# hmc-lair-shark-tracking/auv-sim

Hardware: AMD Instinct MI355X
Metric: RRT-Dubins node expansions/s (RRT.exploring) (higher is better)
Workload: dtype f64; 1 GPU; RRT.exploring 256 obst 200x200 cells 10000 iters x 12288 episodes/GPU, timebin parent sampling; episodes_per_gpu=12288, iters=10000, obstacles=256, cells=40000, parallelism=episodes sharded x1

## Files before the change

auv_sim_amd/csrc/rrt_explore_kernel.h:

```cpp
#ifndef AUVP_RRT_EXPLORE_KERNEL_H
#define AUVP_RRT_EXPLORE_KERNEL_H
#include "auvp_math.h"
#include "auvp_types.h"
#include "auvp_wave.h"

namespace auvp {

constexpr int RRT_WAVES = 4;
constexpr int RRT_X_WAVES = 8;
constexpr int RRT_MAX_CHUNK = 63;
constexpr int RRT_MAX_HAB = 64;
constexpr int RRT_MAX_POLY = 64;
constexpr int RRT_MAX_BINS = 64;
constexpr int RRT_ELIST = 192;

struct RrtTables {
  WorldDev* world;
  RrtParamsDev* params;
  double (*hab)[4];
  double (*poly)[2];
  double (*bins)[2];
};
constexpr int RRT_WORLD_ONLY_BYTES = (int)((sizeof(WorldDev) + 15) & ~(size_t)15);
constexpr int RRT_WORLD_BYTES = RRT_WORLD_ONLY_BYTES + (int)((sizeof(RrtParamsDev) + 15) & ~(size_t)15);
__host__ __device__ inline int rrt_tables_bytes(int n_habitats, int n_poly, int n_bins) {
  return RRT_WORLD_BYTES + n_habitats * 32 + n_poly * 16 + n_bins * 16;
}
__device__ __forceinline__ RrtTables rrt_tables_view(unsigned char* base, int n_habitats, int n_poly) {
  RrtTables t;
  t.world = reinterpret_cast<WorldDev*>(base);
  t.params = reinterpret_cast<RrtParamsDev*>(base + RRT_WORLD_ONLY_BYTES);
  t.hab = reinterpret_cast<double(*)[4]>(base + RRT_WORLD_BYTES);
  t.poly = reinterpret_cast<double(*)[2]>(base + RRT_WORLD_BYTES + n_habitats * 32);
  t.bins = reinterpret_cast<double(*)[2]>(base + RRT_WORLD_BYTES + n_habitats * 32 + n_poly * 16);
  return t;
}
__device__ __forceinline__ void rrt_tables_stage(const RrtTables& S, const WorldDev& W) {
  for (int i = threadIdx.x; i < W.n_habitats; i += blockDim.x) {
    S.hab[i][0] = W.hab[3 * i]; S.hab[i][1] = W.hab[3 * i + 1]; S.hab[i][2] = W.hab[3 * i + 2];
    S.hab[i][3] = W.hab_t[i];
  }
  if (threadIdx.x == 0) *S.world = W;
  for (int i = threadIdx.x; i < W.n_poly * 2; i += blockDim.x) (&S.poly[0][0])[i] = W.poly[i];
  for (int i = threadIdx.x; i < W.n_bins * 2; i += blockDim.x) (&S.bins[0][0])[i] = W.bins[i];
}

struct RrtLdsPlan {
  int chunk;
  int tables, scratch, mt, pts, bins, per_wave, total;
};

__host__ __device__ inline RrtLdsPlan rrt_lds_plan(int K, int max_pts, int nfreq, int obst_slots, int tables_bytes,
                                                   int waves = RRT_X_WAVES) {
  RrtLdsPlan p;
  p.chunk = nfreq < 1 ? 1 : (nfreq > RRT_MAX_CHUNK ? RRT_MAX_CHUNK : nfreq);
  const int C = p.chunk;
  int steer_u = (64 + 3 * C + 3) * 8;
  int steer_s = (7 * ((C + 2) & ~1) + 4) * 8;
  int s = steer_u > steer_s ? steer_u : steer_s;
  p.scratch = (s + 15) & ~15;
  p.mt = 624 * 4;
  p.pts = ((max_pts * 16) + 15) & ~15;
  p.bins = (((K + 2) * 4) + 15) & ~15;
  p.per_wave = p.scratch + p.mt + p.pts + p.bins;
  p.tables = (tables_bytes + 15) & ~15;
  p.total = p.tables + waves * p.per_wave + obst_slots * (3 * 8 + 4);
  return p;
}

__device__ __forceinline__ bool any_point_outside(const double (*poly)[2], int nv, const double (*pts)[2], int n_pts) {
  const int lane = lane_id();
  if (nv <= 0) return n_pts > 0;
  const int per = 64 / nv;
  const int e = lane % nv, pl = lane / nv;
  const int ej = e == 0 ? nv - 1 : e - 1;
  const double xi = poly[e][0], yi = poly[e][1], xj = poly[ej][0], yj = poly[ej][1];
  bool outside = false;
  for (int p0 = 0; p0 < n_pts; p0 += per) {
    const int p = p0 + pl;
    const bool live = pl < per && p < n_pts;
    bool cross = false;
    if (live) {
      const double x = pts[p][0], y = pts[p][1];
      if ((yi > y) != (yj > y)) cross = x < (xj - xi) * (y - yi) / (yj - yi) + xi;
    }
    const unsigned long long cm = wave_ballot(cross);
    const int q = p0 + lane;
    if (lane < per && q < n_pts) {
      const unsigned long long grp = (cm >> (lane * nv)) & (nv == 64 ? ~0ull : ((1ull << nv) - 1ull));
      outside = outside | ((__popcll(grp) & 1) == 0);
    }
  }
  return wave_any(outside);
}

__device__ __forceinline__ int lower_bound_from(const double* __restrict__ a, int n, double v, int i) {
  i = i < 0 ? 0 : (i > n - 1 ? n - 1 : i);
  while (i > 0 && a[i - 1] >= v) i--;
  while (i < n && a[i] < v) i++;
  return i;
}

__device__ __forceinline__ int cell_lookup(const WorldDev& W, double x, double y, const double* grid_lds = nullptr) {
  if (W.n_cells == 0) return -1;
  if (W.sg_enabled && grid_lds) {
    const double *x1 = grid_lds, *x0 = grid_lds + W.sg_ncol, *y1 = x0 + W.sg_ncol, *y0 = y1 + W.sg_nrow;
    int c = (int)auvp_floor((x - W.sg_x1_0) * W.sg_inv_dx) + 1, r = (int)auvp_floor((x - W.sg_y1_0) * W.sg_inv_dy) + 1;
    c = c < 0 ? 0 : (c > W.sg_ncol - 1 ? W.sg_ncol - 1 : c);
    r = r < 0 ? 0 : (r > W.sg_nrow - 1 ? W.sg_nrow - 1 : r);
    const double xc1 = x1[c], xcm = c > 0 ? x1[c - 1] : -__builtin_inf();
    const double yr1 = y1[r], yrm = r > 0 ? y1[r - 1] : -__builtin_inf();
    if (!(xcm < x && xc1 >= x)) c = lower_bound_from(x1, W.sg_ncol, x, c);
    if (!(yrm < x && yr1 >= x)) r = lower_bound_from(y1, W.sg_nrow, x, r);
    if (c >= W.sg_ncol || r >= W.sg_nrow) return -1;
    return (x0[c] <= x && y0[r] <= y) ? r * W.sg_ncol + c : -1;
  }
  if (W.sg_enabled) {
    int gc = (int)auvp_floor((x - W.sg_x1_0) * W.sg_inv_dx) + 1, gr = (int)auvp_floor((x - W.sg_y1_0) * W.sg_inv_dy) + 1;
    gc = gc < 0 ? 0 : (gc > W.sg_ncol - 1 ? W.sg_ncol - 1 : gc);
    gr = gr < 0 ? 0 : (gr > W.sg_nrow - 1 ? W.sg_nrow - 1 : gr);
    const double4 cc = reinterpret_cast<const double4*>(W.sg_col)[gc];
    const double4 rr = reinterpret_cast<const double4*>(W.sg_row)[gr];
    if (cc.x < x && cc.y >= x && rr.x < x && rr.y >= x) return (cc.z <= x && rr.z <= y) ? gr * W.sg_ncol + gc : -1;
    const int c = lower_bound_from(W.sg_x1, W.sg_ncol, x, gc);
    const int r = lower_bound_from(W.sg_y1, W.sg_nrow, x, gr);
    if (c >= W.sg_ncol || r >= W.sg_nrow) return -1;
    if (!(W.sg_x0[c] <= x) || !(W.sg_y0[r] <= y)) return -1;
    return r * W.sg_ncol + c;
  }
  double fb = auvp_floor((x - W.xb_x0) * W.xb_inv_w);
  int b = fb < 0.0 ? 0 : (fb >= (double)W.n_xbuckets ? W.n_xbuckets - 1 : (int)fb);
  if (W.rg_enabled) {
    int lo = W.rg_first[b], hi = W.rg_first[b + 1];
    while (lo < hi) { const int mid = (lo + hi) >> 1; if (W.rg_bp[mid] < x) lo = mid + 1; else hi = mid; }
    const int r = 2 * lo + ((lo < W.n_rg_bp && W.rg_bp[lo] == x) ? 1 : 0);
    const int s = W.rg_off[r], e = W.rg_off[r + 1];
    if (s == e) return -1;
    if (W.rg_pm[s] <= y) return W.rg_id[s];
    if (!(W.rg_pm[e - 1] <= y)) return -1;
    lo = s; hi = e - 1;
    while (hi - lo > 1) { const int mid = (lo + hi) >> 1; if (W.rg_pm[mid] <= y) hi = mid; else lo = mid; }
    return W.rg_id[hi];
  }
  int e = W.xb_off[b + 1];
  for (int k = W.xb_off[b]; k < e; k++) {
    const double4 d = reinterpret_cast<const double4*>(W.xb_data)[k];
    if (y < d.w) return -1;
    if (x >= d.x && x <= d.y && y >= d.z) return W.xb_items[k];
  }
  return -1;
}

struct BinLists {
  int32_t* direct;
  int32_t* over;
  int32_t* dir;
  int n_over, k1;
};

__device__ __forceinline__ BinLists bin_lists(const RrtBuffers& B, size_t episode, int K) {
  BinLists L;
  L.n_over = B.bin_over; L.k1 = K + 1;
  L.direct = B.bin_items + episode * (size_t)B.bin_stride;
  L.over = L.direct + (size_t)L.k1 * AUVP_BIN_HEAD;
  L.dir = L.over + (size_t)L.n_over * 64;
  return L;
}

__device__ __forceinline__ int bin_member(const BinLists& L, int b, int k) {
  if (k < AUVP_BIN_HEAD) return L.direct[b * AUVP_BIN_HEAD + k];
  const int kk = k - AUVP_BIN_HEAD;
  const int chunk = L.dir[(kk >> 6) * L.k1 + b];
  return L.over[chunk * 64 + (kk & 63)];
}

__device__ __forceinline__ int32_t* bin_slot_for_append(const BinLists& L, int b, int c, int& next_chunk, bool writer) {
  if (c < AUVP_BIN_HEAD) return L.direct + (b * AUVP_BIN_HEAD + c);
  const int kk = c - AUVP_BIN_HEAD;
  int32_t* d = L.dir + ((kk >> 6) * L.k1 + b);
  int chunk;
  if ((kk & 63) == 0) {
    if (next_chunk >= L.n_over) return nullptr;
    chunk = next_chunk++;
    if (writer) *d = chunk;
  } else {
    chunk = *d;
  }
  return L.over + (chunk * 64 + (kk & 63));
}

struct CostAcc {
  double c2;
  unsigned long long visited;
  int hits;
};

template <bool LIM = false>
__device__ __forceinline__ void cost_element(const WorldDev& W, const RrtTables& S, int bin_lo, int bin_hi, double w3,
                                             double x, double y, double t, double& tv, int& hab, bool hab_near = true,
                                             const double* grid_lds = nullptr, unsigned long long keep = ~0ull) {
  int tb = -1;
  if (W.bins_sorted) {
    if (bin_hi > bin_lo) {
      int i = (int)auvp_floor((t - W.bins_t1_0) * W.bins_inv_len) + 1;
      i = i < bin_lo ? bin_lo : (i > bin_hi - 1 ? bin_hi - 1 : i);
      const double2 bi = *reinterpret_cast<const double2*>(&S.bins[i][0]);
      const double pm = i > bin_lo ? S.bins[i - 1][1] : -__builtin_inf();
      if (pm < t && bi.y >= t) {
        if (bi.x <= t) tb = i;
      } else {
        while (i > bin_lo && S.bins[i - 1][1] >= t) i--;
        while (i < bin_hi && S.bins[i][1] < t) i++;
        if (i < bin_hi && S.bins[i][0] <= t) tb = i;
      }
    }
  } else {
    for (int b = bin_hi - 1; b >= bin_lo; b--) {
      const double2 r = *reinterpret_cast<const double2*>(&S.bins[b][0]);
      tb = (t >= r.x && t <= r.y) ? b : tb;
    }
  }
  tv = 0.0;
  hab = -1;
  if (tb >= 0) {
    int c = cell_lookup(W, x, y, grid_lds);
    if (c >= 0) tv = w3 * W.prob[(size_t)tb * W.n_cells + c];
    if (hab_near) {
      if (W.hg_n > 0) {
        const double fx = auvp_floor((x - W.hg_x0) * W.hg_inv_w), fy = auvp_floor((y - W.hg_y0) * W.hg_inv_h);
        unsigned long long m = 0ull;
        if (fx >= 0.0 && fy >= 0.0 && fx < (double)W.hg_n && fy < (double)W.hg_n) m = W.hg_mask[(int)fy * W.hg_n + (int)fx];
        if constexpr (LIM) m &= keep;
        while (m) {
          const int h = __ffsll((long long)m) - 1;
          m &= m - 1ull;
          const double2 hxy = *reinterpret_cast<const double2*>(&S.hab[h][0]);
          const double ddx = hxy.x - x, ddy = hxy.y - y;
          if (ddx * ddx + ddy * ddy <= S.hab[h][3]) { hab = h; break; }
        }
      } else {
        for (int h = W.n_habitats - 1; h >= 0; h--) {
          const double2 hxy = *reinterpret_cast<const double2*>(&S.hab[h][0]);
          const double ddx = hxy.x - x, ddy = hxy.y - y;
          if constexpr (LIM) hab = (ddx * ddx + ddy * ddy <= S.hab[h][3] && ((keep >> h) & 1ull)) ? h : hab;
          else hab = (ddx * ddx + ddy * ddy <= S.hab[h][3]) ? h : hab;
        }
      }
    }
  }
}

__device__ __forceinline__ void cost_accumulate(int n_valid, double tv, int hab, double* term, CostAcc& acc) {
  const int lane = lane_id();
  term[lane] = tv;
  unsigned long long hm = wave_ballot(hab >= 0);
  acc.hits += __popcll(hm);
  unsigned long long vis = acc.visited;
  while (hm) {
    int l = __ffsll((long long)hm) - 1;
    int h = __builtin_amdgcn_readlane(hab, l);
    vis |= (1ull << h);
    hm &= ~wave_ballot(hab == h);
  }
  acc.visited = vis;
  wave_sync();
  double c2 = acc.c2;
  for (int i = 0; i < n_valid; i += 8) {
    double2 v[4];
#pragma unroll
    for (int k = 0; k < 4; k++) v[k] = *reinterpret_cast<const double2*>(term + i + 2 * k);
#pragma unroll
    for (int k = 0; k < 4; k++) { c2 = c2 + v[k].x; c2 = c2 + v[k].y; }
  }
  acc.c2 = c2;
  wave_sync();
}

struct CostPre {
  int tb, c, midx;
};
__device__ __forceinline__ CostPre cost_pre(const WorldDev& W, const RrtTables& S, int bin_lo, int bin_hi, double x, double y, double t,
                                            const double* grid_lds) {
  CostPre q;
  q.tb = -1; q.c = -1; q.midx = -1;
  if (W.bins_sorted) {
    if (bin_hi > bin_lo) {
      int i = (int)auvp_floor((t - W.bins_t1_0) * W.bins_inv_len) + 1;
      i = i < bin_lo ? bin_lo : (i > bin_hi - 1 ? bin_hi - 1 : i);
      const double2 bi = *reinterpret_cast<const double2*>(&S.bins[i][0]);
      const double pm = i > bin_lo ? S.bins[i - 1][1] : -__builtin_inf();
      if (pm < t && bi.y >= t) {
        if (bi.x <= t) q.tb = i;
      } else {
        while (i > bin_lo && S.bins[i - 1][1] >= t) i--;
        while (i < bin_hi && S.bins[i][1] < t) i++;
        if (i < bin_hi && S.bins[i][0] <= t) q.tb = i;
      }
    }
  } else {
    for (int b = bin_hi - 1; b >= bin_lo; b--) {
      const double2 r = *reinterpret_cast<const double2*>(&S.bins[b][0]);
      q.tb = (t >= r.x && t <= r.y) ? b : q.tb;
    }
  }
  if (q.tb >= 0) {
    q.c = cell_lookup(W, x, y, grid_lds);
    if (W.hg_n > 0) {
      const double fx = auvp_floor((x - W.hg_x0) * W.hg_inv_w), fy = auvp_floor((y - W.hg_y0) * W.hg_inv_h);
      if (fx >= 0.0 && fy >= 0.0 && fx < (double)W.hg_n && fy < (double)W.hg_n) q.midx = (int)fy * W.hg_n + (int)fx;
    }
  }
  return q;
}
template <bool LIM = false>
__device__ __forceinline__ void cost_post(const WorldDev& W, const RrtTables& S, double w3, double x, double y, const CostPre& q,
                                          double prob, unsigned long long m, double& tv, int& hab, unsigned long long keep = ~0ull) {
  tv = 0.0;
  hab = -1;
  if (q.tb >= 0) {
    if (q.c >= 0) tv = w3 * prob;
    if (W.hg_n > 0) {
      if constexpr (LIM) m &= keep;
      while (m) {
        const int h = __ffsll((long long)m) - 1;
        m &= m - 1ull;
        const double2 hxy = *reinterpret_cast<const double2*>(&S.hab[h][0]);
        const double ddx = hxy.x - x, ddy = hxy.y - y;
        if (ddx * ddx + ddy * ddy <= S.hab[h][3]) { hab = h; break; }
      }
    } else {
      for (int h = W.n_habitats - 1; h >= 0; h--) {
        const double2 hxy = *reinterpret_cast<const double2*>(&S.hab[h][0]);
        const double ddx = hxy.x - x, ddy = hxy.y - y;
        if constexpr (LIM) hab = (ddx * ddx + ddy * ddy <= S.hab[h][3] && ((keep >> h) & 1ull)) ? h : hab;
        else hab = (ddx * ddx + ddy * ddy <= S.hab[h][3]) ? h : hab;
      }
    }
  }
}

__device__ __forceinline__ void cost_pass(const WorldDev& W, const RrtTables& S, int bin_lo, int bin_hi, double w3,
                                          int n_valid, double x, double y, double t, double* term, CostAcc& acc) {
  double tv = 0.0;
  int hab = -1;
  if (lane_id() < n_valid) cost_element(W, S, bin_lo, bin_hi, w3, x, y, t, tv, hab);
  cost_accumulate(n_valid, tv, hab, term, acc);
}

constexpr int RRT_NN_UNROLL = 8;
constexpr int RRT_NN_BLOCK = 64 * RRT_NN_UNROLL;
__host__ __device__ inline long long rrt_nn_stride(int cap_nodes) {
  return ((long long)cap_nodes + RRT_NN_BLOCK - 1) / RRT_NN_BLOCK * RRT_NN_BLOCK;
}

__device__ __forceinline__ int nn_closest(const double2* __restrict__ xy, int n_nodes, double rx, double ry, bool force_exact = false,
                                          int* slow = nullptr) {
  const int lane = lane_id();
  const double inf = __builtin_inf();
  double bd = inf, sd = inf;
  int bt = 0;
  for (int base = 0; base < n_nodes; base += RRT_NN_BLOCK) {
    double2 q[RRT_NN_UNROLL];
#pragma unroll
    for (int u = 0; u < RRT_NN_UNROLL; u++) q[u] = xy[base + u * 64 + lane];
#pragma unroll
    for (int u = 0; u < RRT_NN_UNROLL; u++) {
      const double ddx = rx - q[u].x, ddy = ry - q[u].y;
      const double d2 = ddx * ddx + ddy * ddy;
      const bool lt = d2 < bd;
      sd = (d2 != bd) ? __builtin_fmin(sd, __builtin_fmax(bd, d2)) : sd;
      bd = lt ? d2 : bd;
      bt = lt ? base + u * 64 : bt;
    }
  }
  const double gmin = wave_min_f64(bd);
  const double band = gmin + gmin * 0x1p-49;
  const bool suspect = (bd > gmin && bd <= band) || (sd > gmin && sd <= band);
  int cand = 0x7fffffff;
  const bool exact = wave_any(suspect) || force_exact;
  if (slow) *slow = exact ? 1 : 0;
  if (!exact) {
    const unsigned long long em = wave_ballot(bd == gmin);
    if (__popcll(em) == 1) return uni(__builtin_amdgcn_readlane(bt, __ffsll((long long)em) - 1) + (__ffsll((long long)em) - 1));
    cand = (bd == gmin) ? bt + lane : 0x7fffffff;
  } else {
    double bs = inf;
    for (int m = lane; m < n_nodes; m += 64) {
      const double2 q = xy[m];
      const double ddx = rx - q.x, ddy = ry - q.y;
      const double d = auvp_sqrt(ddx * ddx + ddy * ddy);
      if (d < bs) { bs = d; cand = m; }
    }
    const double smin = wave_min_f64(bs);
    cand = (bs == smin) ? cand : 0x7fffffff;
  }
#pragma unroll
  for (int o = 32; o >= 1; o >>= 1) {
    const int t = __shfl_xor(cand, o, 64);
    cand = t < cand ? t : cand;
  }
  return uni(cand);
}

template <int J, int MODE, bool DIAG>
__global__ __launch_bounds__(RRT_X_WAVES * 64, (MODE == 2 ? (J <= 4 ? 5 : 2) : (J <= 4 ? 6 : 2))) void rrt_explore_kernel(WorldDev W, RrtParamsDev P, RrtBuffers B,
                                                                     int n_episodes, int max_pts) {
  constexpr bool LIM = false;
  constexpr const RrtEpisodeLimDev* lim = nullptr;
#include "rrt_explore_body.h"
}

template <int J>
__global__ __launch_bounds__(RRT_X_WAVES * 64, (J <= 4 ? 6 : 2)) void rrt_explore_lim_kernel(WorldDev W, RrtParamsDev P, RrtBuffers B,
                                                                                           int n_episodes, int max_pts,
                                                                                           const RrtEpisodeLimDev* __restrict__ lim) {
  constexpr int MODE = 0;
  constexpr bool DIAG = false, LIM = true;
#include "rrt_explore_body.h"
}

constexpr int RRT_LEAF_WAVES = 4;
#ifndef AUVP_LEAF_NPL
#define AUVP_LEAF_NPL 2
#endif
#ifndef AUVP_LEAF_WPE
#define AUVP_LEAF_WPE 4
#endif
__host__ __device__ inline int rrt_leaf_grid_lds_bytes(int sg_enabled, int ncol, int nrow) {
  const long long b = 16LL * ((long long)ncol + nrow);
  return (sg_enabled && b <= 48 * 1024) ? (int)b : 0;
}
__host__ __device__ inline int rrt_leaf_mark_words(int cap_nodes) {
  const int w = (cap_nodes + 31) / 32;
  return w <= 4096 ? w : 0;
}

static __global__ __launch_bounds__(RRT_LEAF_WAVES * 64) __attribute__((amdgpu_waves_per_eu(AUVP_LEAF_WPE, AUVP_LEAF_WPE))) void rrt_leaf_kernel(WorldDev W, RrtParamsDev P, RrtBuffers B, int n_episodes,
                                                                      int mark_words) {
  constexpr bool LIM = false;
  constexpr const RrtEpisodeLimDev* lim = nullptr;
#include "rrt_leaf_body.h"
}

static __global__ __launch_bounds__(RRT_LEAF_WAVES * 64) __attribute__((amdgpu_waves_per_eu(AUVP_LEAF_WPE, AUVP_LEAF_WPE))) void rrt_leaf_lim_kernel(
    WorldDev W, RrtParamsDev P, RrtBuffers B, int n_episodes, int mark_words, const RrtEpisodeLimDev* __restrict__ lim) {
  constexpr bool LIM = true;
#include "rrt_leaf_body.h"
}

static __global__ __launch_bounds__(64) void rrt_final_course_kernel(RrtBuffers B, const int64_t* __restrict__ offsets,
                                                              double* __restrict__ out, int n_episodes) {
  const int ep = blockIdx.x;
  if (ep >= n_episodes) return;
  const int lane = lane_id();
  const RrtSummary s = B.summary[ep];
  if (s.best_leaf < 0) return;
  const int capn = B.cap_nodes;
  const size_t capp = (size_t)B.cap_points;
  const double* nodeF = B.node_f + (size_t)ep * capn * 8;
  const int4* nodeI = reinterpret_cast<const int4*>(B.node_i) + (size_t)ep * capn;
  const double* ptF = B.points + (size_t)ep * capp * 6;
  const double* init = B.init + (size_t)ep * 6;
  double* o = out + 7 * (size_t)offsets[ep];
  int pos = s.best_path_len - 1;
  auto node_elem = [&](int m, int at) {
    double* e = o + 7 * (size_t)at;
    const int4 r = nodeI[m];
    if (r.y < 0) {
      e[0] = init[0]; e[1] = init[1]; e[2] = init[2]; e[3] = 0.0; e[4] = init[3]; e[5] = init[4]; e[6] = init[5];
    } else {
      const double* nf = nodeF + (size_t)m * 8;
      e[0] = nf[0]; e[1] = nf[1]; e[2] = nf[2]; e[3] = 0.0; e[4] = nf[3]; e[5] = (double)r.x; e[6] = nf[4];
    }
  };
  if (lane == 0) node_elem(s.best_leaf, pos);
  pos--;
  for (int m = s.best_leaf;;) {
    const int4 r = nodeI[m];
    if (r.y < 0) break;
    const int cnt = r.w, off = r.z;
    for (int k = lane; k < cnt; k += 64) {
      double* e = o + 7 * (size_t)(pos - cnt + 1 + k);
      size_t gi = (size_t)off + k;
      const double* ra = ptF + gi * 3;
      const double* rb = ptF + capp * 3 + gi * 3;
      e[0] = ra[0]; e[1] = ra[1]; e[2] = rb[0]; e[3] = rb[1];
      e[4] = ra[2]; e[5] = (double)r.x; e[6] = rb[2];
    }
    pos -= cnt;
    if (lane == 0) node_elem(r.y, pos);
    pos--;
    m = r.y;
  }
}

}
#endif
```

auv_sim_amd/csrc/rrt_rows_body.h:

```cpp
  extern __shared__ __align__(16) unsigned char smem[];
  const RrtTables S = rrt_tables_view(smem, W.n_habitats, W.n_poly);
  const int wave = (int)(threadIdx.x >> 6);
  const int lane = lane_id();
  const int row = lane >> 4, rl = lane & 15, rowbase = lane & 48;
  const int K = P.K;
  const int wg_waves = (int)(blockDim.x >> 6);
#if AUVP_ROWS_BODY_STREAM
  const RowsStreamLdsPlan plan = rrt_rows_stream_lds_plan(K, RW_MAX_OBST, rrt_tables_bytes(W.n_habitats, W.n_poly, W.n_bins), wg_waves, MIRROR);
  unsigned char* ebase = smem + plan.tables + (size_t)(wave * RW_ROWS + row) * plan.per_ep;
  double* ring = reinterpret_cast<double*>(ebase);
  double* inc = reinterpret_cast<double*>(ebase + plan.ring);
  uint16_t* bin_count = reinterpret_cast<uint16_t*>(ebase + plan.ring + plan.scratch);
#else
  const RowsLdsPlan plan = rrt_rows_lds_plan(K, RW_MAX_OBST, rrt_tables_bytes(W.n_habitats, W.n_poly, W.n_bins), wg_waves);
  unsigned char* ebase = smem + plan.tables + (size_t)(wave * RW_ROWS + row) * plan.per_ep;
  uint32_t* mt = reinterpret_cast<uint32_t*>(ebase);
  double* win = reinterpret_cast<double*>(ebase + plan.mt);
  double* inc = win;
  uint16_t* bin_count = reinterpret_cast<uint16_t*>(ebase + plan.mt + plan.scratch);
#endif

  rrt_tables_stage(S, W);
  if (threadIdx.x == 0) *S.params = P;
  const RrtParamsDev& Q = *S.params;
  double* olx = reinterpret_cast<double*>(smem + plan.tables + (size_t)wg_waves * RW_ROWS * plan.per_ep);
  double* oly = olx + RW_MAX_OBST;
  float* olr = reinterpret_cast<float*>(oly + RW_MAX_OBST);
  for (int i = threadIdx.x; i < RW_MAX_OBST; i += blockDim.x) { olx[i] = W.os_x[i]; oly[i] = W.os_y[i]; olr[i] = W.os_r[i]; }
  __syncthreads();

  const int ep = ((int)blockIdx.x * wg_waves + wave) * RW_ROWS + row;
  bool live = ep < n_episodes;
  const int eps = live ? ep : 0;
  if (!wave_any(live)) return;

  const int capn = B.cap_nodes, capp = B.cap_points, bcap = B.bin_cap;
  double* nodeF = B.node_f + (size_t)eps * capn * 8;
  int4* nodeI = reinterpret_cast<int4*>(B.node_i) + (size_t)eps * capn;
  uint8_t* nodeQ = B.node_q + (size_t)eps * capn;
  double* ptF = B.points + (size_t)eps * capp * 6;
  const BinLists bins = bin_lists(B, (size_t)eps, K);
  int next_chunk = 0;
  const double* init = B.init + (size_t)eps * 6;

#if AUVP_ROWS_BODY_STREAM
  RowStream rng;
  rng.ring = ring;
  rng.src = B.stream + (size_t)eps * (size_t)B.stream_cap;
  rng.pos = 0u; rng.front = 0u; rng.req = 0u;
  rng.cap = (uint32_t)B.stream_cap;
#pragma unroll
  for (int c = 0; c < RS_PEND; c++) rng.pend[c] = rs_piece(0.0);
#ifdef AUVP_STREAM_COUNT_SLOW
  rng.slow = 0u;
#endif
#define ROWS_CONSUME(on, n) stream_advance(rng, on, (uint32_t)(n))
#else
  RowRng rng;
  rng.s = mt;
  for (int i = rl; i < 624; i += 16) mt[i] = B.mt[(size_t)eps * 624 + i];
  {
    int idx = B.mt_index ? B.mt_index[eps] : 624;
    idx = idx < 0 ? 0 : (idx > 624 ? 624 : idx);
    rng.pslot = idx == 624 ? 0u : (uint32_t)idx;
    rng.avail = (uint32_t)(624 - idx);
    rng.drawn = 0ull;
  }
#define ROWS_CONSUME(on, n) rows_advance(rng, on, (uint32_t)(2 * (n)))
#endif
  for (int i = rl; i < K + 2; i += 16) bin_count[i] = 0;
  wave_sync();
  if (live && rl == 0) {
    nodeF[0] = init[0]; nodeF[1] = init[1]; nodeF[2] = init[2]; nodeF[3] = init[3]; nodeF[4] = init[5];
    nodeI[0] = make_int4(0, -1, 0, 0);
    nodeQ[0] = 0;
    bins.direct[(K >= 1 ? 1 : 0) * AUVP_BIN_HEAD] = 0;
    bin_count[K >= 1 ? 1 : 0] = 1;
  }
  wave_sync();
  int n_nodes = 1, n_points = 0, status = 0, n_cand = 0, iters_run = 0;
  double4 sbox_ld = reinterpret_cast<const double4*>(W.os_box)[rl];
  asm volatile("" : "+v"(sbox_ld.x), "+v"(sbox_ld.y), "+v"(sbox_ld.z), "+v"(sbox_ld.w));
  const double4 sbox = sbox_ld;
  typedef const __attribute__((address_space(4))) double* rows_ost_ptr;
  const rows_ost_ptr ost_s = (rows_ost_ptr)W.os_t;
  const int nv_poly = W.n_poly;

  for (int it = 0; it < P.max_iter; it++) {
    if (!wave_any(live)) break;
    int par = 0, n_total = 0, base = 0;
    {
      bool search = live;
      int fo = 0, rb = 0, cnt = 0;
      double u = 0.0;
#if AUVP_ROWS_BODY_STREAM
      StreamBase<MIRROR> sel;
#endif
      for (;;) {
#if AUVP_ROWS_BODY_STREAM
        if (!stream_ensure<MIRROR>(rng, search, 16u, rl) && search) { status = AUVP_ST_STREAM; live = false; iters_run = it; search = false; }
        sel = stream_base<MIRROR>(rng, 0u, rl);
        if (search) u = stream_read(sel, rl, rl);
#else
        rows_ensure(rng, search, 32u, rl);
        if (search) { u = rows_random_at(rng, (uint32_t)rl); win[rl] = u; }
#endif
        const int rbj = (int)py_uniform(1.0, (double)(K + 1), u);
        const bool cand = search && rl < 14;
        const bool badkey = cand && rbj > K;
        const int cj = (cand && !badkey) ? (int)bin_count[rbj] : 0;
        const uint32_t okm = row_ballot(cj != 0, rowbase), badm = row_ballot(badkey, rowbase);
        const int f_ok = okm ? (__ffs((int)okm) - 1) : 16, f_bad = badm ? (__ffs((int)badm) - 1) : 16;
        if (search) {
          if (f_bad < f_ok) { status = -5; live = false; iters_run = it; search = false; }
          else if (f_ok < 16) { fo = f_ok; search = false; }
        }
        const bool again = search;
        ROWS_CONSUME(again, 14);
        const int src = rowbase + (again ? 0 : fo);
        const int rb_n = row_read(rbj, src), cnt_n = row_read(cj, src);
        if (!again && live && cnt == 0) { rb = rb_n; cnt = cnt_n; }
        if (!wave_any(again)) break;
      }
#if AUVP_ROWS_BODY_STREAM
      const double u1 = stream_read(sel, fo + 1, rl), u2 = stream_read(sel, fo + 2, rl);
#else
      wave_sync();
      const double u1 = win[fo + 1], u2 = win[fo + 2];
#endif
      if (live) {
        const int ri = (int)py_uniform(0.0, (double)cnt, u1);
        par = bin_member(bins, rb, ri);
        n_total = (int)auvp_floor(py_uniform(0.0, Q.freq, u2) / 1);
        base = fo + 3;
      }
    }
    const bool on0 = live && 0 < n_total;
    const int n0_ = on0 ? (n_total < RW_C ? n_total : RW_C) : 0;
#if AUVP_ROWS_BODY_STREAM
    if (!stream_ensure<MIRROR>(rng, on0, (uint32_t)(base + 3 * n0_), rl) && on0) { status = AUVP_ST_STREAM; live = false; iters_run = it; }
#else
    auto make_window = [&](bool on, int nwin, int b0) {
      rows_ensure(rng, on, (uint32_t)(2 * (b0 + nwin)), rl);
#pragma unroll
      for (int t = 0; t < 3; t++) {
        const int j = rl + 16 * t;
        if (on && j < nwin) win[j] = rows_random_at(rng, (uint32_t)(b0 + j));
      }
      wave_sync();
    };
    {
      const int e_end = base + 3 * n0_;
      rows_ensure(rng, on0, (uint32_t)(2 * e_end), rl);
#pragma unroll
      for (int t = 0; t < 3; t++) {
        const int e = 16 + rl + 16 * t;
        if (on0 && e < e_end) win[e] = rows_random_at(rng, (uint32_t)e);
      }
      wave_sync();
    }
#endif
    double cx = 0.0, cy = 0.0, cth = 0.0, ctt = 0.0, clen = 0.0;
    if (live) {
      const double2 a = *reinterpret_cast<const double2*>(nodeF + (size_t)par * 8);
      const double2 b = *reinterpret_cast<const double2*>(nodeF + (size_t)par * 8 + 2);
      cx = a.x; cy = a.y; cth = b.x; ctt = b.y;
      clen = nodeF[(size_t)par * 8 + 4];
    }
#if AUVP_ROWS_BODY_STREAM
    stream_top_up<MIRROR>(rng, live, rl);
#endif
    const double px0 = cx, py0 = cy, clen0 = clen;
    int cnt = 0;
    double ptx[2] = {0.0, 0.0}, pty[2] = {0.0, 0.0};
    bool ptv[2] = {false, false};
    bool first_pass = true;
#pragma unroll
    for (int pass = 0; pass < 2; pass++) {
      const int c0 = pass * RW_C;
      const bool on = live && c0 < n_total;
      if (pass != 0 && !wave_any(on)) break;
      const int n = on ? ((n_total - c0) < RW_C ? (n_total - c0) : RW_C) : 0;
      const int nwin = 3 * n;
#ifdef AUVP_ROWS_PAD
      {
        double pd0 = cth, pd1 = cx, pd2 = cy, pd3 = ctt;
#pragma unroll
        for (int q = 0; q < AUVP_ROWS_PAD / 4; q++)
          asm volatile("v_add_f64 %0, %0, 1.0\n\tv_add_f64 %1, %1, 1.0\n\tv_add_f64 %2, %2, 1.0\n\tv_add_f64 %3, %3, 1.0"
                       : "+v"(pd0), "+v"(pd1), "+v"(pd2), "+v"(pd3));
      }
#endif
      const int b0 = first_pass ? base : 0;
#if AUVP_ROWS_BODY_STREAM
      if (pass != 0 && !stream_ensure<MIRROR>(rng, on, (uint32_t)nwin, rl) && on) { status = AUVP_ST_STREAM; live = false; iters_run = it; }
      const StreamBase<MIRROR> wb = stream_base<MIRROR>(rng, (uint32_t)b0, rl);
#define ROWS_WIN(j) stream_read(wb, (j), rl)
#else
      if (pass != 0) make_window(on, nwin, b0);
      const double* wp = win + (pass == 0 ? base : 0);
#define ROWS_WIN(j) wp[j]
#endif
      unsigned long long tpred = 0ull;
#pragma unroll
      for (int t = 0; t < 3; t++) {
        const int j = rl + 16 * t;
        const double dist = py_uniform(0.0, Q.dist_to_end, ROWS_WIN(j));
        const double diff = py_uniform(-Q.diff_max, Q.diff_max, ROWS_WIN(j + 1));
        const unsigned long long fb = __builtin_amdgcn_fcmp(auvp_fabs(dist), auvp_fabs(diff), 2 ) &
                                      __builtin_amdgcn_uicmp((unsigned)(j + 1), (unsigned)nwin, 36 );
        tpred |= ((fb >> rowbase) & 0xffffull) << (16 * t);
      }
      const bool active = rl < n;
      const uint32_t mywin = active ? (uint32_t)(tpred >> (2 * rl)) : 0u;
      const uint32_t below_me = active ? ((1u << rl) - 1u) : 0u;
      int cbelow = active ? rl : 0;
      uint32_t tmask;
      for (;;) {
        const unsigned long long tb = __builtin_amdgcn_uicmp((mywin >> cbelow) & 1u, 0u, 33 );
        tmask = (uint32_t)((tb >> rowbase) & 0xffffull);
        const int cnew = __popc(tmask & below_me);
        const unsigned long long chg = __builtin_amdgcn_uicmp((unsigned)cnew, (unsigned)cbelow, 33 );
        cbelow = cnew;
        if (chg == 0ull) break;
      }
      const int mypos = 2 * rl + cbelow;
      const int used = 2 * n + __popc(tmask);
      const bool taken = (tmask >> rl) & 1u;
      double radius = 0.0, phi = 0.0, vt = 1.0;
      if (taken) {
        const double dist = py_uniform(0.0, Q.dist_to_end, ROWS_WIN(mypos));
        const double diff = py_uniform(-Q.diff_max, Q.diff_max, ROWS_WIN(mypos + 1));
        const double s1 = dist + diff, s2 = dist - diff;
        radius = auvp_div_plain(s1 + s2, -s1 + s2);
        phi = auvp_div_plain(s1 + s2, 2 * radius);
        vt = py_uniform(0.0, 2 * Q.v, ROWS_WIN(mypos + 2));
      }
#undef ROWS_WIN
#if !AUVP_ROWS_BODY_STREAM
      wave_sync();
#endif
      inc[rl] = phi;
      wave_sync();
      const double th = rows_theta_chain(cth, inc);
      const double myth = (rl == 15) ? cth : th;
      double sn, cs;
      auvp_sincos_sk(myth, &sn, &cs);
      double dx = 0.0, dy = 0.0, mv = 0.0, dt = 0.0;
      {
        const uint32_t below = tmask & ((1u << rl) - 1u);
        const int prev = below ? (31 - __clz((int)below)) : 15;
        const double so = row_read_f64(sn, rowbase + prev), co = row_read_f64(cs, rowbase + prev);
        if (taken) {
          dx = radius * (sn - so);
          dy = radius * (-cs + co);
          mv = auvp_sqrt_plain(dx * dx + dy * dy);
          dt = auvp_div_plain(mv, vt);
        }
      }
      if (rl < 15) { inc[rl] = dx; inc[18 + rl] = dy; inc[36 + rl] = dt; inc[54 + rl] = mv; }
      else { inc[15] = 0.0; inc[33] = 0.0; inc[51] = 0.0; inc[69] = 0.0; }
      wave_sync();
      if (rl < 4 && on) {
        double acc = rl == 0 ? cx : (rl == 1 ? cy : (rl == 2 ? ctt : clen));
        double2* rowp = reinterpret_cast<double2*>(inc + rl * 18);
        double2 v[8];
#pragma unroll
        for (int s2 = 0; s2 < 8; s2++) v[s2] = rowp[s2];
#pragma unroll
        for (int s2 = 0; s2 < 8; s2++) { acc = acc + v[s2].x; v[s2].x = acc; acc = acc + v[s2].y; v[s2].y = acc; }
#pragma unroll
        for (int s2 = 0; s2 < 8; s2++) rowp[s2] = v[s2];
      }
      wave_sync();
      double mx = 0.0, my = 0.0, mt_ = 0.0, ml = 0.0;
      if (active) { mx = inc[rl]; my = inc[18 + rl]; mt_ = inc[36 + rl]; ml = inc[54 + rl]; }
      const bool app = taken && (mv >= Q.min_dist);
      const uint32_t amask = row_ballot(app, rowbase);
      const int napp = __popc(amask);
      if (on && (n_points + cnt + napp > capp)) { status = -2; live = false; iters_run = it; }
      const bool wr = app && live;
      if (wr) {
        const int rank = __popc(amask & ((1u << rl) - 1u));
        const size_t gi = (size_t)(n_points + cnt + rank);
        double* ra = ptF + gi * 3;
        double* rb = ptF + (size_t)capp * 3 + gi * 3;
        typedef double nt_f64x2 __attribute__((ext_vector_type(2)));
        nt_f64x2 va, vb; va.x = mx; va.y = my; vb.x = myth; vb.y = vt;
        __builtin_nontemporal_store(va, reinterpret_cast<nt_f64x2*>(ra)); __builtin_nontemporal_store(mt_, ra + 2);
        __builtin_nontemporal_store(vb, reinterpret_cast<nt_f64x2*>(rb)); __builtin_nontemporal_store(ml, rb + 2);
      }
      ptx[pass] = mx; pty[pass] = my; ptv[pass] = wr;
      {
        const int last = n > 0 ? n - 1 : 0;
        const double th_last = row_read_f64(myth, rowbase + last);
        if (on) {
          cnt += napp;
          cx = inc[last]; cy = inc[18 + last]; ctt = inc[36 + last]; clen = inc[54 + last];
          cth = th_last;
        }
      }
      ROWS_CONSUME(on && live, b0 + used);
      first_pass = false;
      wave_sync();
    }
    ROWS_CONSUME(live && n_total == 0, base);

    const double reach = clen - clen0;
    const double bx0 = px0 - reach, by0 = py0 - reach, bx1 = px0 + reach, by1 = py0 + reach;
    const double slack = 0x1p-30 * (auvp_fabs(bx0) + auvp_fabs(bx1) + auvp_fabs(by0) + auvp_fabs(by1) + 1.0);
    const double hx = reach + slack;
    bool hit = false;
    double ex0 = bx0, ey0 = by0, ex1 = bx1, ey1 = by1;
    auto cull_and_test = [&](auto tight_tag) {
      constexpr bool TIGHT = decltype(tight_tag)::value;
      const double hs = hx + slack;
      const bool slot_hit = live && !(sbox.z < px0 - hs || sbox.x > px0 + hs || sbox.w < py0 - hs || sbox.y > py0 + hs);
      uint32_t sm = row_ballot(slot_hit, rowbase);
      double tcx = px0, tcy = py0, thx = hx, thy = hx;
      if (TIGHT) {
        double mnx = px0, mxx = px0, mny = py0, mxy = py0;
#pragma unroll
        for (int q = 0; q < 2; q++) {
          if (ptv[q]) {
            mnx = __builtin_fmin(mnx, ptx[q]); mxx = __builtin_fmax(mxx, ptx[q]);
            mny = __builtin_fmin(mny, pty[q]); mxy = __builtin_fmax(mxy, pty[q]);
          }
        }
        mnx = row_min_f64(mnx); mxx = row_max_f64(mxx); mny = row_min_f64(mny); mxy = row_max_f64(mxy);
        const double ts = 0x1p-30 * (auvp_fabs(mnx) + auvp_fabs(mxx) + auvp_fabs(mny) + auvp_fabs(mxy) + 1.0);
        tcx = (mnx + mxx) * 0.5; tcy = (mny + mxy) * 0.5;
        thx = (mxx - mnx) * 0.5 + ts; thy = (mxy - mny) * 0.5 + ts;
        const bool tight = slot_hit && !(sbox.z < mnx - ts || sbox.x > mxx + ts || sbox.w < mny - ts || sbox.y > mxy + ts);
        sm = row_ballot(tight, rowbase);
        ex0 = mnx; ey0 = mny; ex1 = mxx; ey1 = mxy;
      }
      while (wave_any(sm != 0u)) {
        const bool hs_ = sm != 0u;
        const int j0 = hs_ ? 16 * (__ffs((int)sm) - 1) : 0;
        sm &= sm - 1u;
        const int oi = j0 + rl;
        const double oxj = olx[oi], oyj = oly[oi], orj = (double)olr[oi];
#ifdef AUVP_ROWS_OST_LDS
        const double otj = orj * orj;
#endif
        const bool cand = hs_ && (TIGHT ? !(auvp_fabs(oxj - tcx) > thx + orj || auvp_fabs(oyj - tcy) > thy + orj)
                                        : !(auvp_fabs(oxj - px0) > hx + orj || auvp_fabs(oyj - py0) > hx + orj));
        uint32_t cm = row_ballot(cand, rowbase);
        n_cand += __popc(cm);
        while (wave_any(cm != 0u)) {
          const bool has = cm != 0u;
          const int cl = has ? (__ffs((int)cm) - 1) : 0;
          cm &= cm - 1u;
          const double ox = row_read_f64(oxj, rowbase + cl), oy = row_read_f64(oyj, rowbase + cl);
#ifdef AUVP_ROWS_OST_LDS
          const double ot = row_read_f64(otj, rowbase + cl);
#else
          const int oc = j0 + cl;
          const unsigned long long hasm = __builtin_amdgcn_uicmp((unsigned)has, 0u, 33 );
          double ot = 0.0;
          int rowv = row;
          asm volatile("" : "+v"(rowv));
#pragma unroll
          for (int r = 0; r < RW_ROWS; r++)
            if (hasm & (1ull << (16 * r))) {
              const double t = ost_s[__builtin_amdgcn_readlane(oc, 16 * r)];
              ot = rowv == r ? t : ot;
            }
#endif
#pragma unroll
          for (int q = 0; q < 2; q++) {
            const double ddx = ptx[q] - ox, ddy = pty[q] - oy;
            hit |= has && ptv[q] && (ddx * ddx + ddy * ddy <= ot);
          }
          if (rl == 15) { const double ddx = px0 - ox, ddy = py0 - oy; hit |= has && (ddx * ddx + ddy * ddy <= ot); }
          if (row_ballot(hit, rowbase) != 0u) cm = 0u;
        }
      }
    };
    if (P.flags & AUVP_KFLAG_TIGHT_CULL) cull_and_test(std::true_type{});
    else cull_and_test(std::false_type{});
    const double* sb = S.world->safe_box;
    const bool box_inside = W.has_safe_box && ex0 > sb[0] && ey0 > sb[1] && ex1 < sb[2] && ey1 < sb[3];
    bool outside = false;
    if (wave_any(live && !box_inside)) {
      auto crossing_outside = [&](double x, double y) {
        if (nv_poly <= 0) return true;
        int par_ = 0;
        for (int e = 0; e < nv_poly; e++) {
          const int ej = e == 0 ? nv_poly - 1 : e - 1;
          const double xi = S.poly[e][0], yi = S.poly[e][1], xj = S.poly[ej][0], yj = S.poly[ej][1];
          if ((yi > y) != (yj > y)) par_ ^= (x < (xj - xi) * (y - yi) / (yj - yi) + xi) ? 1 : 0;
        }
        return (par_ & 1) == 0;
      };
      const bool need = live && !box_inside;
#pragma unroll
      for (int q = 0; q < 2; q++)
        if (need && ptv[q]) outside |= crossing_outside(ptx[q], pty[q]);
      if (need && rl == 15) outside |= crossing_outside(px0, py0);
    }
    const bool bad = row_ballot(hit || outside, rowbase) != 0u;
    const bool ok = live && !bad;
    if (ok && n_nodes >= capn) { status = -2; live = false; iters_run = it; }
    const bool acc_ = ok && live;
    const int me = n_nodes;
    if (acc_) {
      double q = auvp_floor(ctt * Q.inv_bin_interval);
      const double r = auvp_fma(-q, Q.bin_interval, ctt);
      if (r < 0.0) q -= 1.0;
      else if (r >= Q.bin_interval) q += 1.0;
      const double fi = q + 1.0;
      const double curr_bin = fi * Q.bin_interval;
      const bool over = curr_bin > Q.max_traj_time;
      bool stored = true;
      if (!over || fi <= (double)K) {
        const int bi = (int)fi;
        const int c = over ? 0 : (int)bin_count[bi];
        int32_t* slot = (c >= bcap || c >= 65535) ? nullptr : bin_slot_for_append(bins, bi, c, next_chunk, rl == 0);
        if (!slot) { status = -2; live = false; iters_run = it; stored = false; }
        else if (rl == 0) { *slot = me; bin_count[bi] = (uint16_t)(c + 1); }
      }
      if (stored) {
        if (rl == 0) {
          double* nf = nodeF + (size_t)me * 8;
          *reinterpret_cast<double2*>(nf) = make_double2(cx, cy);
          *reinterpret_cast<double2*>(nf + 2) = make_double2(cth, ctt);
          nf[4] = clen;
          nodeI[me] = make_int4(it, par, n_points, cnt);
          nodeQ[me] = ctt >= Q.max_traj_time - 30 ? 1 : 0;
        }
        n_nodes++;
        n_points += cnt;
      }
    }
    wave_sync();
  }

  const bool valid = ep < n_episodes;
  if (live) iters_run = P.max_iter;
#if AUVP_ROWS_BODY_STREAM
  const unsigned long long drawn = 2ull * rng.pos;
  if (!stream_ensure<MIRROR>(rng, valid && status == 0, 1u, rl) && valid && status == 0) status = AUVP_ST_STREAM;
  const double after = status == AUVP_ST_STREAM ? 0.0 : stream_read(stream_base<MIRROR>(rng, 0u, rl), rl, rl);
#else
  const unsigned long long drawn = rng.drawn;
  rows_ensure(rng, valid, 2u, rl);
  const double after = rows_random_at(rng, 0u);
#endif
  if (valid) {
    for (int i = rl; i < K + 1; i += 16) B.bin_count[(size_t)ep * (K + 1) + i] = (int32_t)bin_count[i];
    if (rl == 0) {
      RrtSummary& s = B.summary[ep];
#if AUVP_ROWS_BODY_STREAM
      pipe_report(B.pipe_fail, status == AUVP_ST_STREAM ? AUVP_ST_PIPELINE : 0);
#endif
      s.status = status; s.n_nodes = n_nodes; s.n_points = n_points; s.n_leaves = 0;
      s.best_leaf = -1; s.best_path_len = 0; s.iters_run = iters_run; s.n_candidates = n_cand;
      s.best_cost[0] = __builtin_inf(); s.best_cost[1] = 0.0; s.best_cost[2] = 0.0; s.best_cost[3] = 0.0;
      s.best_length = 0.0;
      s.rng_after = after; s.leaf_elems = 0; s.n_draw32 = drawn; s.nn_scanned = 0ull;
#if AUVP_ROWS_BODY_STREAM && defined(AUVP_STREAM_COUNT_SLOW)
      s.nn_scanned = rng.slow;
#endif
    }
  }
#undef ROWS_CONSUME
```

auv_sim_amd/csrc/rrt_rows_stream_kernel.h:

```cpp
#ifndef AUVP_RRT_ROWS_STREAM_KERNEL_H
#define AUVP_RRT_ROWS_STREAM_KERNEL_H
#include "rrt_rows_kernel.h"

namespace auvp {

constexpr int RS_RING = 256;
constexpr int RS_MIRROR = 48;
constexpr int RS_WAVES = 16;
#ifndef AUVP_RS_PIECE
#define AUVP_RS_PIECE 2
#endif
constexpr int RS_PIECE = AUVP_RS_PIECE;
constexpr int RS_CHUNK = 16 * RS_PIECE;
constexpr int RS_PEND = 64 / RS_CHUNK;
typedef double rs_f64x2 __attribute__((ext_vector_type(2)));
template <int N> struct RsPiece { typedef double type; };
template <> struct RsPiece<2> { typedef rs_f64x2 type; };
typedef RsPiece<RS_PIECE>::type rs_piece;
constexpr int RS_LDS_LIMIT = 160 * 1024;

struct RowsStreamLdsPlan {
  int tables, ring, scratch, bins, per_ep, obst, total;
};
__host__ __device__ inline RowsStreamLdsPlan rrt_rows_stream_lds_plan(int K, int n_obst_slots, int tables_bytes, int waves = RW_WAVES, bool mirror = false) {
  RowsStreamLdsPlan p;
  p.tables = (tables_bytes + 15) & ~15;
  p.ring = (RS_RING + (mirror ? RS_MIRROR : 0)) * 8;
  p.scratch = (4 * 18 * 8 + 15) & ~15;
  p.bins = (((K + 2) * 2) + 15) & ~15;
  p.per_ep = p.ring + p.scratch + p.bins;
  p.obst = n_obst_slots * (8 + 8 + 4);
  p.total = p.tables + waves * RW_ROWS * p.per_ep + p.obst;
  return p;
}

struct RowsStreamShape {
  int waves;
  bool mirror;
  RowsStreamLdsPlan plan;
};
__host__ inline RowsStreamShape rrt_rows_stream_shape(int K, int n_obst_slots, int tables_bytes, int waves_wanted, int force = -1) {
  int sw = waves_wanted < 1 ? 1 : (waves_wanted > RW_WAVES ? RW_WAVES : waves_wanted);
  while (sw > 1 && rrt_rows_stream_lds_plan(K, n_obst_slots, tables_bytes, sw, false).total > RS_LDS_LIMIT) sw--;
  bool mirror = force < 0 ? rrt_rows_stream_lds_plan(K, n_obst_slots, tables_bytes, sw, true).total <= RS_LDS_LIMIT : force != 0;
  while (mirror && sw > 1 && rrt_rows_stream_lds_plan(K, n_obst_slots, tables_bytes, sw, true).total > RS_LDS_LIMIT) sw--;
  RowsStreamShape s;
  s.waves = sw; s.mirror = mirror;
  s.plan = rrt_rows_stream_lds_plan(K, n_obst_slots, tables_bytes, sw, mirror);
  return s;
}

struct RowStream {
  double* ring;
  const double* src;
  uint32_t pos, front, req, cap;
  rs_piece pend[RS_PEND];
#ifdef AUVP_STREAM_COUNT_SLOW
  uint32_t slow;
#endif
};

template <bool MIRROR>
__device__ __forceinline__ void stream_commit(RowStream& r, int rl) {
#pragma unroll
  for (int c = 0; c < RS_PEND; c++)
    if (r.front + (uint32_t)(RS_CHUNK * c) < r.req) {
      const uint32_t s = (r.front + (uint32_t)(RS_CHUNK * c) + (uint32_t)(RS_PIECE * rl)) & (uint32_t)(RS_RING - 1);
      *reinterpret_cast<rs_piece*>(r.ring + s) = r.pend[c];
      if (MIRROR && s < (uint32_t)RS_MIRROR) *reinterpret_cast<rs_piece*>(r.ring + s + (uint32_t)RS_RING) = r.pend[c];
    }
  r.front = r.req;
}
__device__ __forceinline__ void stream_request(RowStream& r, bool on, int rl) {
  const uint32_t room = (uint32_t)RS_RING - (r.front - r.pos), left = r.cap - r.req;
  uint32_t n = (room < left ? room : left) / (uint32_t)RS_CHUNK;
  n = n > (uint32_t)RS_PEND ? (uint32_t)RS_PEND : n;
  n = on ? n : 0u;
#pragma unroll
  for (int c = 0; c < RS_PEND; c++)
    if ((uint32_t)c < n)
      r.pend[c] = __builtin_nontemporal_load(reinterpret_cast<const rs_piece*>(r.src + r.req + (uint32_t)(RS_CHUNK * c) + (uint32_t)(RS_PIECE * rl)));
  r.req += (uint32_t)RS_CHUNK * n;
}
__device__ __forceinline__ void stream_settle(RowStream& r) {
#pragma unroll
  for (int c = 0; c < RS_PEND; c++) asm volatile("" : "+v"(r.pend[c]));
}
template <bool MIRROR>
__device__ __forceinline__ void stream_top_up(RowStream& r, bool on, int rl) {
  stream_commit<MIRROR>(r, rl);
  stream_request(r, on, rl);
}
template <bool MIRROR>
__device__ __forceinline__ bool stream_ensure(RowStream& r, bool want, uint32_t need, int rl) {
  const uint32_t need_w = want ? need : 0u;
  const bool ok = r.pos + need_w <= r.cap;
  for (;;) {
    if (__builtin_amdgcn_uicmp(r.front - r.pos, ok ? need_w : 0u, 36 ) == 0ull) break;
    const bool go = ok && r.front - r.pos < need_w;
#ifdef AUVP_STREAM_COUNT_SLOW
    if (go) r.slow++;
#endif
    stream_commit<MIRROR>(r, rl);
    stream_request(r, go && ok, rl);
    stream_commit<MIRROR>(r, rl);
    stream_settle(r);
    wave_sync();
    if (!wave_any(go && ok && r.front - r.pos < need_w)) break;
  }
  wave_sync();
  return ok;
}
template <bool MIRROR> struct StreamBase;
template <> struct StreamBase<true> { const double* p; };
template <> struct StreamBase<false> { const double* ring; uint32_t first; };
template <bool MIRROR>
__device__ __forceinline__ StreamBase<MIRROR> stream_base(const RowStream& r, uint32_t b, int rl) {
  if constexpr (MIRROR) return StreamBase<true>{r.ring + (((r.pos + b) & (uint32_t)(RS_RING - 1)) + (uint32_t)rl)};
  else return StreamBase<false>{r.ring, r.pos + b};
}
__device__ __forceinline__ double stream_read(const StreamBase<true>& w, int j, int rl) { return w.p[j - rl]; }
__device__ __forceinline__ double stream_read(const StreamBase<false>& w, int j, int) { return w.ring[(w.first + (uint32_t)j) & (uint32_t)(RS_RING - 1)]; }
__device__ __forceinline__ void stream_advance(RowStream& r, bool on, uint32_t n) {
  if (on) r.pos += n;
}

template <int MAXW>
static __global__ __launch_bounds__(MAXW * 64, 1) void rrt_rows_stream_kernel(WorldDev W, RrtParamsDev P, RrtBuffers B, int n_episodes) {
  constexpr bool MIRROR = true;
#define AUVP_ROWS_BODY_STREAM 1
#include "rrt_rows_body.h"
#undef AUVP_ROWS_BODY_STREAM
}
template <int MAXW>
static __global__ __launch_bounds__(MAXW * 64, 1) void rrt_rows_stream_masked_kernel(WorldDev W, RrtParamsDev P, RrtBuffers B, int n_episodes) {
  constexpr bool MIRROR = false;
#define AUVP_ROWS_BODY_STREAM 1
#include "rrt_rows_body.h"
#undef AUVP_ROWS_BODY_STREAM
}

}
#endif
```

Before: 1.356 billion expansions/s.

## Speculatively pre-sample next iteration's parent during current expansion in stream kernel

In the streaming RRT kernel, right after consuming the current iteration's randoms, the next iteration's bin/parent selection is computed early from data already in the ring, and the bin-list word load is started so it overlaps the collision-check work. The speculation is cancelled if the chosen bin is appended to or becomes non-empty, or if the episode dies, in which case the normal search loop runs. A compiler barrier on the chunk load in append keeps ordering. This adds register pressure and duplicated ballot/row-read work per iteration, and it risks divergence when some rows fall back to the search loop.

```diff
diff --git a/auv_sim_amd/csrc/rrt_explore_kernel.h b/auv_sim_amd/csrc/rrt_explore_kernel.h
--- a/auv_sim_amd/csrc/rrt_explore_kernel.h
+++ b/auv_sim_amd/csrc/rrt_explore_kernel.h
@@ -174,6 +174,7 @@
   return L.over[chunk * 64 + (kk & 63)];
 }
 
+template <bool SETTLE = false>
 __device__ __forceinline__ int32_t* bin_slot_for_append(const BinLists& L, int b, int c, int& next_chunk, bool writer) {
   if (c < AUVP_BIN_HEAD) return L.direct + (b * AUVP_BIN_HEAD + c);
   const int kk = c - AUVP_BIN_HEAD;
@@ -185,6 +186,7 @@
     if (writer) *d = chunk;
   } else {
     chunk = *d;
+    if constexpr (SETTLE) asm volatile("" : "+v"(chunk));
   }
   return L.over + (chunk * 64 + (kk & 63));
 }
diff --git a/auv_sim_amd/csrc/rrt_rows_body.h b/auv_sim_amd/csrc/rrt_rows_body.h
--- a/auv_sim_amd/csrc/rrt_rows_body.h
+++ b/auv_sim_amd/csrc/rrt_rows_body.h
@@ -85,12 +85,33 @@
   typedef const __attribute__((address_space(4))) double* rows_ost_ptr;
   const rows_ost_ptr ost_s = (rows_ost_ptr)W.os_t;
   const int nv_poly = W.n_poly;
+#if AUVP_ROWS_BODY_STREAM
+  int sp_word = 0, sp_nt = 0, sp_rb = 0, sp_key = 0;
+#ifdef AUVP_SPEC_COUNT_FALLBACK
+  uint32_t sp_fallbacks = 0u;
+#endif
+#endif
 
   for (int it = 0; it < P.max_iter; it++) {
     if (!wave_any(live)) break;
     int par = 0, n_total = 0, base = 0;
+#if AUVP_ROWS_BODY_STREAM
+    const bool searching = live && sp_key == 0;
+#define ROWS_SEARCHING searching
+    if (live && sp_key != 0) {
+      n_total = sp_nt; base = sp_key & 31;
+      par = sp_word;
+      if (sp_key & 0x10000) par = bins.over[par * 64 + ((sp_key >> 8) & 63)];
+    }
+#ifdef AUVP_SPEC_COUNT_FALLBACK
+    if (wave_any(searching) && live) sp_fallbacks++;
+#endif
+    if (wave_any(searching))
+#else
+#define ROWS_SEARCHING live
+#endif
     {
-      bool search = live;
+      bool search = ROWS_SEARCHING;
       int fo = 0, rb = 0, cnt = 0;
       double u = 0.0;
 #if AUVP_ROWS_BODY_STREAM
@@ -128,13 +149,14 @@
       wave_sync();
       const double u1 = win[fo + 1], u2 = win[fo + 2];
 #endif
-      if (live) {
+      if (ROWS_SEARCHING && live) {
         const int ri = (int)py_uniform(0.0, (double)cnt, u1);
         par = bin_member(bins, rb, ri);
         n_total = (int)auvp_floor(py_uniform(0.0, Q.freq, u2) / 1);
         base = fo + 3;
       }
     }
+#undef ROWS_SEARCHING
     const bool on0 = live && 0 < n_total;
     const int n0_ = on0 ? (n_total < RW_C ? n_total : RW_C) : 0;
 #if AUVP_ROWS_BODY_STREAM
@@ -305,6 +327,36 @@
       wave_sync();
     }
     ROWS_CONSUME(live && n_total == 0, base);
+#if AUVP_ROWS_BODY_STREAM
+    sp_key = 0;
+    if (it + 1 < P.max_iter) {
+      const bool sp_on = live && stream_holds(rng, 16u);
+      const StreamBase<MIRROR> ssel = stream_base<MIRROR>(rng, 0u, rl);
+      double su = 0.0;
+      if (sp_on) su = stream_read(ssel, rl, rl);
+      const int rbj = (int)py_uniform(1.0, (double)(K + 1), su);
+      const bool cand = sp_on && rl < 14;
+      const bool badkey = cand && rbj > K;
+      const int cj = (cand && !badkey) ? (int)bin_count[rbj] : 0;
+      const uint32_t okm = row_ballot(cj != 0, rowbase), badm = row_ballot(badkey, rowbase);
+      const int f_ok = okm ? (__ffs((int)okm) - 1) : 16, f_bad = badm ? (__ffs((int)badm) - 1) : 16;
+      const bool holds = sp_on && f_ok < 16 && f_ok < f_bad;
+      const int fo = holds ? f_ok : 0;
+      const int rb_n = row_read(rbj, rowbase + fo), cnt_n = row_read(cj, rowbase + fo);
+      const double u1 = stream_read(ssel, fo + 1, rl), u2 = stream_read(ssel, fo + 2, rl);
+      if (holds) {
+        const int ri = (int)py_uniform(0.0, (double)cnt_n, u1);
+        if (ri < AUVP_BIN_HEAD) { sp_word = bins.direct[rb_n * AUVP_BIN_HEAD + ri]; sp_key = fo + 3; }
+        else {
+          const int kk = ri - AUVP_BIN_HEAD;
+          sp_word = bins.dir[(kk >> 6) * bins.k1 + rb_n];
+          sp_key = (fo + 3) | ((kk & 63) << 8) | 0x10000;
+        }
+        sp_nt = (int)auvp_floor(py_uniform(0.0, Q.freq, u2) / 1);
+        sp_rb = rb_n;
+      }
+    }
+#endif
 
     const double reach = clen - clen0;
     const double bx0 = px0 - reach, by0 = py0 - reach, bx1 = px0 + reach, by1 = py0 + reach;
@@ -416,8 +468,18 @@
       bool stored = true;
       if (!over || fi <= (double)K) {
         const int bi = (int)fi;
+#if AUVP_ROWS_BODY_STREAM
+        const int cb = (int)bin_count[bi];
+        if (bi == sp_rb || cb == 0) sp_key = 0;
+        const int c = over ? 0 : cb;
+#else
         const int c = over ? 0 : (int)bin_count[bi];
+#endif
+#if AUVP_ROWS_BODY_STREAM
+        int32_t* slot = (c >= bcap || c >= 65535) ? nullptr : bin_slot_for_append<true>(bins, bi, c, next_chunk, rl == 0);
+#else
         int32_t* slot = (c >= bcap || c >= 65535) ? nullptr : bin_slot_for_append(bins, bi, c, next_chunk, rl == 0);
+#endif
         if (!slot) { status = -2; live = false; iters_run = it; stored = false; }
         else if (rl == 0) { *slot = me; bin_count[bi] = (uint16_t)(c + 1); }
       }
@@ -434,6 +496,9 @@
         n_points += cnt;
       }
     }
+#if AUVP_ROWS_BODY_STREAM
+    if (!live) sp_key = 0;
+#endif
     wave_sync();
   }
 
@@ -463,6 +528,9 @@
 #if AUVP_ROWS_BODY_STREAM && defined(AUVP_STREAM_COUNT_SLOW)
       s.nn_scanned = rng.slow;
 #endif
+#if AUVP_ROWS_BODY_STREAM && defined(AUVP_SPEC_COUNT_FALLBACK)
+      s.nn_scanned = sp_fallbacks;
+#endif
     }
   }
 #undef ROWS_CONSUME
diff --git a/auv_sim_amd/csrc/rrt_rows_stream_kernel.h b/auv_sim_amd/csrc/rrt_rows_stream_kernel.h
--- a/auv_sim_amd/csrc/rrt_rows_stream_kernel.h
+++ b/auv_sim_amd/csrc/rrt_rows_stream_kernel.h
@@ -124,6 +124,9 @@
 __device__ __forceinline__ void stream_advance(RowStream& r, bool on, uint32_t n) {
   if (on) r.pos += n;
 }
+__device__ __forceinline__ bool stream_holds(const RowStream& r, uint32_t n) {
+  return r.front - r.pos >= n && r.pos + n <= r.cap;
+}
 
 template <int MAXW>
 static __global__ __launch_bounds__(MAXW * 64, 1) void rrt_rows_stream_kernel(WorldDev W, RrtParamsDev P, RrtBuffers B, int n_episodes) {
```

After: 1.363 billion expansions/s (median of 6 runs). About the same (+0.5%).
